# lujiarui/esmdiff

Hardware: AMD Instinct MI355X
Metric: conformation samples/sec (256-res, 25 steps) (higher is better)
Workload: dtype bf16

## Files before the change

esmdiff_amd/_native.py:

```python
from __future__ import annotations

import ctypes
from pathlib import Path

import os

_LIB_PATH = Path(os.environ.get("ESMDIFF_LIB") or Path(__file__).resolve().parent / "lib" / "libesmdiff_hip.so")
_lib = None

c_f32p = ctypes.POINTER(ctypes.c_float)
c_i64p = ctypes.POINTER(ctypes.c_int64)

EPI_BF16, EPI_RESID_F32, EPI_SWIGLU_BF16, EPI_BIAS_GELU_BF16, EPI_BIAS_F32 = range(5)
DT_F32, DT_BF16 = 0, 1
PRECISION = {"bf16": 0, "f32": 1, "f32_split": 2, "f16": 3}
F32EPI_STORE, F32EPI_BIAS_GELU, F32EPI_RESID_DIV = range(3)
SECTIONS = ["embed", "layernorm", "gemm_qkv", "qk_norm_rope", "attention", "gemm_out", "gemm_ffn_up",
            "gemm_ffn_down", "head", "sampler"]


class Config(ctypes.Structure):
    _fields_ = [("d_model", ctypes.c_int32), ("n_heads", ctypes.c_int32), ("n_layers", ctypes.c_int32),
                ("ffn_hidden", ctypes.c_int32), ("vocab_out", ctypes.c_int32), ("freq_dim", ctypes.c_int32),
                ("max_batch", ctypes.c_int32), ("max_len", ctypes.c_int32), ("residue_scale", ctypes.c_float),
# ... 29 lines not shown
    "esmdiff_attention_f16", "esmdiff_qk_norm_rope", "esmdiff_add_layernorm", "esmdiff_geom_attention",
    "esmdiff_set_lengths", "esmdiff_attention_ragged", "esmdiff_attention_16_parts",
    "esmdiff_q_xt", "esmdiff_nelbo_rows", "esmdiff_nelbo_eval",
    "esmdiff_superpose_pairs", "esmdiff_tm_pairs",
    "esmdiff_cluster_threshold", "esmdiff_cluster_gromos",
    "esmdiff_lddt_pairs",
    "esmdiff_flex_pair_msf", "esmdiff_flex_fit", "esmdiff_flex_moments",
    "esmdiff_dssp",
    "esmdiff_contact_map", "esmdiff_native_contacts",
    "esmdiff_backbone_torsions", "esmdiff_ramachandran",
    "esmdiff_shape_frames", "esmdiff_debye_frames",
    "esmdiff_describe_gemm_choice", "esmdiff_gemm_workspace_floats",
    "esmdiff_dim6_to_backbone", "esmdiff_plddt_mean", "esmdiff_pair_features", "esmdiff_pae_tm",
    "esmdiff_decoder_set_pair_chunk_bytes",
    "esmdiff_encoder_knn", "esmdiff_encoder_neighbourhood", "esmdiff_encoder_nearest_code",
    "esmdiff_forward_logits_needed", "esmdiff_get_tail_rows",
    "esmdiff_layernorm_f32rows", "esmdiff_swiglu_f32", "esmdiff_qk_norm_rope_f32", "esmdiff_v_split",
    "esmdiff_attention_f32_parts", "esmdiff_gemm_split_k", "esmdiff_get_attention_scales",
    "esmdiff_convert_weight", "esmdiff_interleave_swiglu", "esmdiff_split_weight_from", "esmdiff_weight_rownorm_max",
    "esmdiff_embed_rows", "esmdiff_gather_table_rows", "esmdiff_sigma_mlp", "esmdiff_layernorm_16in",
    "esmdiff_mask_row_list", "esmdiff_gather_rows16", "esmdiff_add_layernorm_rows", "esmdiff_copy_masked_logits",
    "esmdiff_ddpm_step_mapped", "esmdiff_move_token_rows", "esmdiff_samples_with_mask", "esmdiff_rows_identical",
]
LDDT_MAX_L, LDDT_MAX_THRESHOLDS = 4096, 8
DSSP_MAX_L = 4096
TM_MAX_L = 1280
CONTACT_MAX_L, CONTACT_TILE, CONTACT_MAX_CHUNKS = 4096, 64, 256
RAMA_MAX_BINS = 72
SHAPE_MAX_L, SHAPE_MAX_BINS = 4096, 4096
DEBYE_MAX_Q, DEBYE_Q_CHUNK = 1024, 8

CLUSTER_MAX_N = 16384
QXT_PHILOX_COLUMN = 4104
OPT_STREAMS, OPT_DUAL_MIN_TOKENS, OPT_NEEDED_ROWS = 1, 2, 3


def flex_pair_slots(n: int) -> int:
    rows = (n + 1) // 2
    return 4 * rows * min(16, max(1, 2048 // rows))


def contact_pair_tiles(L: int) -> int:
    tiles = (L + CONTACT_TILE - 1) // CONTACT_TILE
    return tiles * (tiles + 1) // 2


def contact_chunk_frames(n: int, L: int) -> int:
    cap = min(CONTACT_MAX_CHUNKS, max(1, 1024 // contact_pair_tiles(L)))
    return max(16, (n + cap - 1) // cap)
# ... 43 lines not shown
            "esmdiff_amd has no CPU fallback.")
    L = ctypes.CDLL(str(_LIB_PATH))
    vp, i32, f32 = ctypes.c_void_p, ctypes.c_int32, ctypes.c_float
    L.esmdiff_abi_version.restype = ctypes.c_int
    L.esmdiff_engine_create.argtypes = [ctypes.POINTER(Config), ctypes.POINTER(Weight), i32, i32,
                                        ctypes.POINTER(vp)]
    L.esmdiff_engine_destroy.argtypes = [vp]
    L.esmdiff_engine_destroy.restype = None
    L.esmdiff_last_error.argtypes = [vp]
    L.esmdiff_last_error.restype = ctypes.c_char_p
    L.esmdiff_forward_logits.argtypes = [vp, vp, vp, vp, vp, i32, i32, i32, vp]
    L.esmdiff_forward_logits_sigmas.argtypes = [vp, vp, vp, vp, vp, i32, i32, i32, vp]
    L.esmdiff_forward_logits_sigmas.restype = ctypes.c_int
    L.esmdiff_forward_logits_needed.argtypes = [vp, vp, vp, vp, vp, i32, i32, i32, vp]
    L.esmdiff_get_tail_rows.argtypes = [vp, c_i64p, i32]
    L.esmdiff_ddpm_step.argtypes = [vp, vp, vp, i32, f32, f32, i32, vp, ctypes.POINTER(Rng), i32, i32, i32, vp]
    L.esmdiff_ddpm_step_margin.argtypes = [vp, vp, vp, i32, f32, f32, i32, ctypes.POINTER(Rng), i32, i32, i32, f32, vp, vp]
    L.esmdiff_ddpm_step_margin.restype = ctypes.c_int
    L.esmdiff_ddpm_step_rows.argtypes = [vp, vp, vp, i32, vp, ctypes.c_uint64, i32, i32, f32, f32, vp, vp, vp]
    L.esmdiff_logit_error_stats.argtypes = [vp, i32, vp, i32, vp, i32, i32, i32, vp, vp]
    L.esmdiff_gibbs_step_rows.argtypes = [vp, vp, vp, vp, i32, f32, f32, vp, ctypes.c_uint64, i32, i32, f32, f32, vp, vp, vp]
    L.esmdiff_get_build_info.argtypes = [ctypes.c_char_p, i32]
    L.esmdiff_describe_plan.argtypes = [vp, i32, i32, ctypes.c_char_p, i32]
    L.esmdiff_set_option.argtypes = [vp, i32, ctypes.c_int64]
    L.esmdiff_ddpm_sample.argtypes = [vp, vp, vp, i32, i32, i32, c_f32p, c_f32p, c_f32p, ctypes.POINTER(Rng), vp]
    L.esmdiff_gibbs_step.argtypes = [vp, vp, vp, vp, i32, f32, f32, vp, vp, ctypes.POINTER(Rng), i32, i32, i32, vp]
    L.esmdiff_gibbs_sample.argtypes = [vp, vp, vp, i32, i32, i32, f32, f32, ctypes.POINTER(i32), ctypes.POINTER(Rng), vp]
    L.esmdiff_gemm_bf16.argtypes = [vp, vp, vp, vp, i32, i32, i32, i32, i32, f32, i32, vp]
    L.esmdiff_gemm_f16.argtypes = [vp, vp, vp, vp, i32, i32, i32, i32, i32, f32, i32, vp]
    if hasattr(L, "esmdiff_gemm_bf16_timed"):
# ... 120 lines not shown
```

esmdiff_amd/csrc/engine.h:

```cpp
#pragma once
#include <math.h>
#include <stdarg.h>
#include <stdio.h>
#include <stdlib.h>
#include <string.h>

#include <algorithm>
#include <map>
#include <string>
#include <vector>

#include "kernels.h"
#define ed ed16
#include "kernels_typed.inc"
#undef ed

#define ED_KN(f16, call) ((f16) ? ed16::call : ed::call)

namespace eng {

enum Section { S_EMBED = 0, S_LN, S_QKV, S_QKROPE, S_ATTN, S_OUT, S_FFN_UP, S_FFN_DOWN, S_HEAD, S_SAMPLER, S_COUNT };

constexpr int64_t kDefaultPairChunkBytes = 1536ll << 20;

// ... 89 lines not shown
        *fmid = nullptr, *fpair_qk = nullptr;
  int step0_share = 0;
  int32_t* flag_dev = nullptr;
  int final_skip = 0;
  int32_t *has_dev = nullptr, *idx_dev = nullptr;
  int64_t *cx = nullptr, *cseq = nullptr;
  float* n_rowloss = nullptr;
  int g_strategy = 0;
  uint32_t* g_inv_mask = nullptr;
  bool g_inv_on = false;
  int needed_rows = 1;
  int32_t *rows_list = nullptr, *rows_map = nullptr, *rows_count = nullptr;
  hipEvent_t ev_rows = nullptr;
  bool rows_mapped = false;
  int64_t stat_tail_rows = 0;
  int64_t stat_forwards = 0, stat_rows = 0;
  int last_B = 0, last_L = 0;
  bool last_pending_delta = false;
  int profiling = 0;
  std::vector<hipEvent_t> ev;
  std::vector<int> ev_section;
  size_t ev_used = 0;
  float prof_ms[16] = {0};
  int prof_launches[16] = {0};
};

namespace eng {

int fail(Owner* o, int code, const char* fmt, ...);
const char* last_error(const Owner* o);
int round_up(int v, int m);
void softplus_host(float* v, int n);
int check_bl(esmdiff_engine* e, int B, int L);
int check_lens(esmdiff_engine* e, int B, int L);
int check_not_decoder(esmdiff_engine* e);
int forward(esmdiff_engine* e, const int64_t* seq, const int64_t* xtok, const float* t_freq_dev, float* logits, int ld, int B, int L,
            hipStream_t st, bool needed_rows = false);
int shared_forward_batch(const esmdiff_engine* e, int B, int L);

#define HIP_TRY(e, call)                                                                              \
  do {                                                                                                \
    hipError_t _s = (call);                                                                           \
    if (_s != hipSuccess) return eng::fail(e, ESMDIFF_E_HIP, "%s: %s", #call, hipGetErrorString(_s)); \
  } while (0)

template <typename T>
int dalloc(Owner* o, T** p, size_t n_elems, bool zero = false) {
  void* v = nullptr;
  hipError_t s = hipMalloc(&v, n_elems * sizeof(T) + 256);
  if (s != hipSuccess) return fail(o, ESMDIFF_E_HIP, "hipMalloc(%zu): %s", n_elems * sizeof(T), hipGetErrorString(s));
  if (zero) hipMemset(v, 0, n_elems * sizeof(T) + 256);
  o->allocs.push_back(v);
// ... 49 lines not shown
```

esmdiff_amd/csrc/engine.hip:

```cpp
#include "engine.h"

using namespace ed;
using namespace eng;

namespace {

thread_local std::string g_error;

}

namespace eng {

int fail(Owner* o, int code, const char* fmt, ...) {
  char buf[512];
  va_list ap;
  va_start(ap, fmt);
  vsnprintf(buf, sizeof buf, fmt, ap);
  va_end(ap);
  if (o) o->err = buf; else g_error = buf;
  return code;
}

const char* last_error(const Owner* o) { return o ? o->err.c_str() : g_error.c_str(); }

// ... 121 lines not shown
    case ESMDIFF_OPT_STREAMS:
      if (value < 1 || value > 4) return fail(e, ESMDIFF_E_INVALID, "ESMDIFF_OPT_STREAMS: 1 .. 4, got %lld", (long long)value);
      HIP_TRY(e, hipSetDevice(e->device));
      while ((int64_t)e->side.size() + 1 < value)
        if (int r = add_side_stream(e)) return r;
      e->n_streams = (int)value;
      return 0;
    case ESMDIFF_OPT_DUAL_MIN_TOKENS:
      if (value < 1) return fail(e, ESMDIFF_E_INVALID, "ESMDIFF_OPT_DUAL_MIN_TOKENS must be positive");
      e->dual_min_tokens = value;
      return 0;
    case ESMDIFF_OPT_NEEDED_ROWS:
      if (value != 0 && value != 1) return fail(e, ESMDIFF_E_INVALID, "ESMDIFF_OPT_NEEDED_ROWS: 0 or 1, got %lld", (long long)value);
      e->needed_rows = (int)value;
      return 0;
    default:
      return fail(e, ESMDIFF_E_INVALID, "unknown option %d", option);
  }
}

int esmdiff_get_build_info(char* buf, int32_t cap) {
#ifdef ED_DEBUG
  const int dbg = 1;
#else
  const int dbg = 0;
#endif
  char tmp[512];
  const int n = snprintf(tmp, sizeof tmp,
                         "libesmdiff_hip abi=%d arch=gfx950 debug_env=%d (%s) operand_builds=bf16,f16 fp_contract_off=sampler,gibbs,metrics "
                         "compiler=%s",
// ... 23 lines not shown
  return 0;
}

int esmdiff_get_counters(esmdiff_engine* e, int64_t* forwards, int64_t* token_rows, int32_t reset) {
  if (!e) return ESMDIFF_E_INVALID;
  if (forwards) *forwards = e->stat_forwards;
  if (token_rows) *token_rows = e->stat_rows;
  if (reset) e->stat_forwards = e->stat_rows = 0;
  return 0;
}

int esmdiff_get_tail_rows(esmdiff_engine* e, int64_t* rows_out, int32_t reset) {
  if (!e) return ESMDIFF_E_INVALID;
  if (rows_out) *rows_out = e->stat_tail_rows;
  if (reset) e->stat_tail_rows = 0;
  return 0;
}

int esmdiff_abi_version(void) { return ESMDIFF_ABI_VERSION; }

const char* esmdiff_last_error(const esmdiff_engine* eng) { return last_error(eng); }

void esmdiff_engine_destroy(esmdiff_engine* e) {
  if (!e) return;
  hipSetDevice(e->device);
  hipDeviceSynchronize();
  for (void* p : e->allocs) hipFree(p);
  for (void* p : {(void*)e->pair_x, (void*)e->pair_h, (void*)e->pair_logits})
    if (p) hipFree(p);
  for (hipEvent_t ev : e->ev) hipEventDestroy(ev);
// ... 258 lines not shown
      TRY(dalloc(e, &e->f_trans, Mx * 3));
      TRY(dalloc(e, &e->f_mask, Mx));
    }
    if (!strict) TRY(dalloc(e, &e->mid, Mx * FH));
    TRY(dalloc(e, &e->logits, Mx * e->ld_logits));
    if (e->has_plddt) TRY(dalloc(e, &e->pl_logits, Mx * e->ld_plddt));
    if (e->has_pair) {
      if (!strict) TRY(dalloc(e, &e->pair_qk, Mx * 128));
      TRY(dalloc(e, &e->tm_rows, Mx));
      TRY(dalloc(e, &e->ptm_dev, (size_t)cfg->max_batch));
    }
    TRY(dalloc(e, &e->cond, (size_t)cfg->max_batch * D));
    TRY(dalloc(e, &e->sig_hidden, (size_t)cfg->max_batch * D));
    e->tfreq_rows = 1026;
    TRY(dalloc(e, &e->tfreq, (size_t)e->tfreq_rows * F));
    TRY(dalloc(e, &e->g_entropy, Mx));
    TRY(dalloc(e, &e->flag_dev, (size_t)4));
    TRY(dalloc(e, &e->has_dev, (size_t)cfg->max_batch));
    TRY(dalloc(e, &e->idx_dev, (size_t)cfg->max_batch));
    TRY(dalloc(e, &e->lens_dev, (size_t)cfg->max_batch));
    TRY(dalloc(e, &e->lens_sub_dev, (size_t)cfg->max_batch));
    TRY(dalloc(e, &e->cx, Mx));
    TRY(dalloc(e, &e->cseq, Mx));
    TRY(dalloc(e, &e->n_rowloss, Mx));
    TRY(dalloc(e, &e->g_inv_mask, (size_t)128, true));
    TRY(dalloc(e, &e->g_sampled, Mx));
    TRY(dalloc(e, &e->g_rowflag, Mx));
    TRY(dalloc(e, &e->g_rowgap, Mx));
    TRY(dalloc(e, &e->g_nunmask, (size_t)e->tfreq_rows * cfg->max_batch));
    {
// ... 116 lines not shown
```

esmdiff_amd/csrc/engine_forward.hip:

```cpp
#include "engine.h"

using namespace ed;
using namespace eng;

namespace {

struct Part {
  const int64_t *seq, *xtok;
  float *x, *logits, *pl_logits;
  bf16_t *h, *h2, *qkv, *q, *k, *ctx, *mid, *dlt, *dlt2, *gp, *gctx, *pair_qk;
  float *fh, *fh2, *fqkv, *fq, *fk, *fctx, *fgu, *fmid, *fgp, *fgctx, *fpair_qk;
  uint16_t* a2;
  float* rs;
  const float *f_rot, *f_trans;
  const uint8_t* f_mask;
  const int32_t* lens;
  int b0, B;
  hipStream_t st;
  const GemmWorkspace *gws, *gws2;
};

void cut_batch(esmdiff_engine* e, Part* parts, int np, const int64_t* seq, const int64_t* xtok, float* logits, int ld, int B, int L,
               hipStream_t st) {
  const int64_t D = e->cfg.d_model, FH = e->cfg.ffn_hidden, VH = e->v_heads;
// ... 295 lines not shown
const char kStaleRows[] =
    "the last forward ran inside esmdiff_ddpm_sample on the rows that hold MASK only (ESMDIFF_OPT_NEEDED_ROWS): the other rows' "
    "hidden state is stale; run a full forward (esmdiff_forward_logits) first, or set the option to 0";

}

int eng::shared_forward_batch(const esmdiff_engine* e, int B, int L) {
  if (e->strict) return 1;
  if (plan_small(e, B, L)) return B;
  for (int b = 1; b < B; ++b)
    if (!plan_small(e, b, L) && (int64_t)b * L >= ed::small_max_rows()) return b;
  return B;
}

int eng::forward(esmdiff_engine* e, const int64_t* seq, const int64_t* xtok, const float* t_freq_dev, float* logits,
                 int ld, int B, int L, hipStream_t st, bool needed_rows) {
  e->last_B = B;
  e->last_L = L;
  e->last_pending_delta = false;
  e->rows_mapped = false;
  e->stat_forwards += 1;
  e->stat_rows += (int64_t)B * L;
  if (e->has_geom && e->frames_B > 0 && (e->frames_B != B || e->frames_L != L))
    return fail(e, ESMDIFF_E_INVALID, "frames were set for B=%d L=%d, forward called with B=%d L=%d", e->frames_B, e->frames_L, B, L);
  const int D = e->cfg.d_model;
  Prof p{e, st};
  const float* cond = nullptr;
  if (t_freq_dev && e->sig_w1) {
    RUN(S_EMBED, launch_sigma_mlp(t_freq_dev, e->sig_w1, e->sig_b1, e->sig_w2, e->sig_b2, e->sig_hidden, e->cond, e->cfg.freq_dim, D, st,
                                  e->sigma_rows));
    cond = e->cond;
  }
  const BatchPlan plan = plan_batch(e, B, L);
  Part parts[4];
  cut_batch(e, parts, plan.np, seq, xtok, logits, ld, B, L, st);
  bool needed = needed_rows && e->needed_rows && e->rows_count && !e->head_split && !plan.small && !e->has_plddt && !e->has_pair &&
                e->cfg.n_layers >= 2;
  if (needed) {
    hipStreamCaptureStatus cs = hipStreamCaptureStatusNone;
    HIP_TRY(e, hipStreamIsCapturing(st, &cs));
    needed = cs == hipStreamCaptureStatusNone;
  }
  if (needed) {
    HIP_TRY(e, launch_mask_row_list(xtok, B, L, plan.np, e->rows_list, e->rows_map, e->rows_count, st));
    HIP_TRY(e, hipEventRecord(e->ev_rows, st));
  }
  if (int r = fork_streams(e, st, plan.np)) return r;
  if (e->strict) {
    for (int pi = 0; pi < plan.np; ++pi)
      if (int r = strict_part(e, parts[pi], cond && e->sigma_rows > 1 ? cond + (int64_t)parts[pi].b0 * D : cond, ld, L)) return r;
  } else if (int r = forward_16bit(e, parts, plan, cond, ld, L, needed)) {
    return r;
  }
  if (!needed) e->stat_tail_rows += (int64_t)B * L;
  return join_streams(e, st, plan.np);
}

extern "C" {

int esmdiff_describe_plan(const esmdiff_engine* e, int32_t B, int32_t L, char* buf, int32_t cap) {
  if (!e || B <= 0 || L <= 0) return ESMDIFF_E_INVALID;
  const esmdiff_config& c = e->cfg;
  const int D = c.d_model, FH = c.ffn_hidden;
  char tmp[1536];
  int n = 0;
  auto room = [&]() { return n < (int)sizeof tmp ? sizeof tmp - (size_t)n : (size_t)0; };
  auto at = [&]() { return tmp + (n < (int)sizeof tmp ? n : (int)sizeof tmp - 1); };
  const char* prec = e->strict ? (e->split ? "f32_split" : "f32") : (e->f16 ? "f16" : "bf16");
  n += snprintf(at(), room(), "precision=%s head=%s B=%d L=%d", prec, (e->strict || e->head_split) ? "f32-grade" : prec, B, L);
  const int np = plan_parts(e, B, L);
// ... 7 lines not shown
    char g1[32], g2[32], g3[32], g4[32];
    const size_t wsf = e->gemm_ws[0].partial ? e->gemm_ws[0].partial_floats : 0;
    ed::describe_gemm(m0, 3 * D, D, wsf, g1, sizeof g1);
    ed::describe_gemm(m0, D, D, wsf, g2, sizeof g2);
    ed::describe_gemm(m0, 2 * FH, D, wsf, g3, sizeof g3);
    ed::describe_gemm(m0, D, FH, 0, g4, sizeof g4);
    n += snprintf(at(), room(), " streams=%d rows_per_stream=%d path=%s", np, m0, small ? "small-batch(K-slice planes summed by the LayerNorm)" : "regular");
    if (small)
      n += snprintf(at(), room(), " gemm[qkv]=%s gemm[out]=128x*/S%d gemm[ffn_up]=%s gemm[ffn_down]=128x*/S%d", g1, ed::gemm_partial_splits(D, D), g3,
                    ed::gemm_partial_splits(D, FH));
    else
      n += snprintf(at(), room(), " gemm[qkv]=%s gemm[out]=%s gemm[ffn_up]=%s gemm[ffn_down]=%s", g1, g2, g3, g4);
  }
  n += snprintf(at(), room(), " step0_sharing=%d final_skip=%d small_max_rows=%d needed_rows=%d", e->step0_share, e->final_skip,
                ed::small_max_rows(), e->needed_rows);
  if (e->lens_B == B) {
    int64_t valid = 0;
    for (int b = 0; b < B; ++b) valid += std::min<int64_t>(e->lens_host[b], L);
    n += snprintf(at(), room(), " ragged=1 valid_tokens=%lld padded_tokens=%lld", (long long)valid, (long long)B * L);
  }
  if (buf && cap > 0) snprintf(buf, (size_t)cap, "%s", tmp);
  return n;
}

int esmdiff_shared_forward_batch(const esmdiff_engine* e, int32_t B, int32_t L) {
  if (!e || B <= 0 || L <= 0 || B > e->cfg.max_batch || L > e->cfg.max_len) return ESMDIFF_E_INVALID;
  return shared_forward_batch(e, B, L);
}

int esmdiff_forward_logits(esmdiff_engine* e, const int64_t* seq, const int64_t* x, const float* t_freq,
// ... 71 lines not shown
```

esmdiff_amd/csrc/engine_sample.hip:

```cpp
#include "engine.h"

using namespace ed;
using namespace eng;

namespace {

int step0_shared_batch(esmdiff_engine* e, const int64_t* seq, const int64_t* x, int B, int L, hipStream_t st, int* shared) {
  *shared = 0;
  if (!e->step0_share || B < 2) return 0;
  if (e->frames_B != 0) return 0;
  if (e->lens_B != 0) return 0;
  const int bs = shared_forward_batch(e, B, L);
  if (bs >= B) return 0;
  HIP_TRY(e, launch_rows_identical(seq, x, B, L, e->flag_dev, st));
  int32_t h = 0;
  HIP_TRY(e, hipMemcpyAsync(&h, e->flag_dev, sizeof h, hipMemcpyDeviceToHost, st));
  HIP_TRY(e, hipStreamSynchronize(st));
  if (h != 0) *shared = bs;
  return 0;
}

int check_mask_head(esmdiff_engine* e, const char* who) {
  return e->cfg.vocab_out <= ESMDIFF_MASK_ID ? fail(e, ESMDIFF_E_INVALID, "%s needs the 4101-way head (mask column)", who) : 0;
}
// ... 123 lines not shown
                        void* stream) {
  if (!e) return ESMDIFF_E_INVALID;
  if (int r = check_not_decoder(e)) return r;
  if (!seq || !x_inout || !mc_t || !mc_s || !rng) return fail(e, ESMDIFF_E_INVALID, "null pointer");
  if (T <= 0 || T + 1 > e->tfreq_rows) return fail(e, ESMDIFF_E_INVALID, "num_steps %d out of range (1..%d)", T, e->tfreq_rows - 1);
  if (e->cfg.time_conditioning && !t_freq) return fail(e, ESMDIFF_E_INVALID, "t_freq required with time conditioning");
  if (int r = check_bl(e, B, L)) return r;
  if (int r = check_lens(e, B, L)) return r;
  hipStream_t st = (hipStream_t)stream;
  const int F = e->cfg.freq_dim;
  if (t_freq) {
    e->tfreq_host.assign(t_freq, t_freq + (size_t)(T + 1) * F);
    HIP_TRY(e, hipMemcpyAsync(e->tfreq, e->tfreq_host.data(), e->tfreq_host.size() * sizeof(float), hipMemcpyHostToDevice, st));
  }
  Prof p{e, st};
  int shared = 0;
  if (int r = step0_shared_batch(e, seq, x_inout, B, L, st, &shared)) return r;
  for (int i = 0; i <= T; ++i) {
    const int Bf = (i == 0 && shared) ? shared : B;
    if (i == T && e->final_skip && T > 0) {
      HIP_TRY(e, launch_samples_with_mask(x_inout, B, L, e->has_dev, st));
      std::vector<int32_t> has(B);
      HIP_TRY(e, hipMemcpyAsync(has.data(), e->has_dev, (size_t)B * 4, hipMemcpyDeviceToHost, st));
      HIP_TRY(e, hipStreamSynchronize(st));
      std::vector<int32_t> idx;
      for (int b = 0; b < B; ++b)
        if (has[b]) idx.push_back(b);
      const int n_live = (int)idx.size();
      if (n_live == 0) break;
      const int n_min = shared_forward_batch(e, B, L);
      if (n_min < B && n_live < B) {
        for (int b = 0; (int)idx.size() < n_min && b < B; ++b)
          if (!has[b]) idx.push_back(b);
        const int n_run = (int)idx.size();
        HIP_TRY(e, hipMemcpyAsync(e->idx_dev, idx.data(), (size_t)n_run * 4, hipMemcpyHostToDevice, st));
        HIP_TRY(e, launch_move_token_rows(x_inout, e->cx, e->idx_dev, n_run, L, 1, st));
        HIP_TRY(e, launch_move_token_rows(seq, e->cseq, e->idx_dev, n_run, L, 1, st));
        std::vector<int32_t> sub_lens;
        if (e->lens_B) {
          for (int j = 0; j < n_run; ++j) sub_lens.push_back(e->lens_host[idx[j]]);
          HIP_TRY(e, hipMemcpyAsync(e->lens_sub_dev, sub_lens.data(), (size_t)n_run * 4, hipMemcpyHostToDevice, st));
          e->cur_lens = e->lens_sub_dev;
        }
        const int rf = forward(e, e->cseq, e->cx, t_freq ? e->tfreq + (size_t)i * F : nullptr, e->logits, e->ld_logits, n_run, L, st, true);
        e->cur_lens = e->lens_B ? e->lens_dev : nullptr;
        if (rf) return rf;
        RUN(S_SAMPLER, launch_ddpm_step(e->cx, e->logits, e->ld_logits, e->cfg.vocab_out, 0.f, 0.f, 1, nullptr, 1, rng->seed, rng->sample_offset, i, n_run, L, st, 0,
                                        0.f, nullptr, e->rows_mapped ? e->rows_map : nullptr));
        HIP_TRY(e, launch_move_token_rows(e->cx, x_inout, e->idx_dev, n_live, L, 0, st));
        HIP_TRY(e, hipStreamSynchronize(st));
        break;
      }
    }
    if (int r = forward(e, seq, x_inout, t_freq ? e->tfreq + (size_t)i * F : nullptr, e->logits, e->ld_logits, Bf, L, st, true)) return r;
    const int fin = i == T;
    RUN(S_SAMPLER, launch_ddpm_step(x_inout, e->logits, e->ld_logits, e->cfg.vocab_out, fin ? 0.f : mc_t[i], fin ? 0.f : mc_s[i],
                                    fin, nullptr, 1, rng->seed, rng->sample_offset, i, B, L, st, Bf < B ? Bf : 0, 0.f, nullptr,
                                    e->rows_mapped ? e->rows_map : nullptr));
  }
  return 0;
}

int esmdiff_gibbs_step(esmdiff_engine* e, int64_t* x_inout, const int64_t* seq, const float* logits, int32_t ld_logits,
                       float temperature, float top_p, const int32_t* n_unmask, const float* u, const esmdiff_rng* rng,
                       int32_t step, int32_t B, int32_t L, void* stream) {
  if (!e) return ESMDIFF_E_INVALID;
  if (!x_inout || !seq || !logits || !n_unmask) return fail(e, ESMDIFF_E_INVALID, "null pointer");
  if (!u && !rng) return fail(e, ESMDIFF_E_INVALID, "need explicit uniforms or an rng");
  if (int r = check_gibbs_filter(e, temperature, top_p, &ld_logits)) return r;
  if (int r = check_bl(e, B, L)) return r;
  if (e->g_strategy == 1 && u) return fail(e, ESMDIFF_E_INVALID, "strategy \"random\" draws its positions from the Philox source: pass rng, not explicit uniforms");
  Prof p{e, (hipStream_t)stream};
  RUN(S_SAMPLER, launch_gibbs_step(x_inout, seq, logits, ld_logits, e->cfg.vocab_out, temperature, top_p, n_unmask, u, u ? 0 : 1, rng ? rng->seed : 0,
// ... 52 lines not shown
```

esmdiff_amd/csrc/kernels.h:

```cpp
#pragma once
#include <stdlib.h>
#include <hip/hip_runtime.h>
#include <stdint.h>

#include "../../include/esmdiff_hip.h"
#include "../../include/esmdiff_hip_test.h"

#include <map>
#include <mutex>
#include <utility>

typedef uint16_t bf16_t;

struct EdGemmWorkspace {
  float* partial;
  size_t partial_floats;
};
struct EdGemmPartials {
  const float* p;
  int S;
  int64_t stride;
};

inline int finish_entry(hipStream_t st) {
// ... 19 lines not shown

hipError_t launch_ddpm_step(int64_t* x, const float* logits, int ld, int V, float mc_t, float mc_s, int final_,
                            const float* u, int use_philox, uint64_t seed, uint64_t sample_offset, int step,
                            int B, int L, hipStream_t stream, int logits_period = 0, float margin = 0.f,
                            int32_t* sample_flags = nullptr, const int32_t* row_map = nullptr);
hipError_t launch_ddpm_step_rows(int64_t* x, const float* logits, int ld, int V, const esmdiff_sample_step* sp, uint64_t seed,
                                 int B, int L, float margin_ratio, float margin_diff, int32_t* sample_flags, float* sample_gap,
                                 hipStream_t stream);
hipError_t launch_logit_error_stats(const float* a, int lda, const float* b, int ldb, const int64_t* x, int rows, int V, int all_columns,
                                    float* out, hipStream_t stream);
hipError_t launch_samples_with_mask(const int64_t* x, int B, int L, int32_t* has, hipStream_t stream);
hipError_t launch_move_token_rows(const int64_t* src, int64_t* dst, const int32_t* idx, int n, int L, int gather, hipStream_t stream);
hipError_t launch_rows_identical(const int64_t* seq, const int64_t* x, int B, int L, int32_t* flag, hipStream_t stream);
__host__ __device__ inline bool needed_rows_compact(int count, int rows) { return (int64_t)count * 8 <= (int64_t)rows * 7; }
hipError_t launch_mask_row_list(const int64_t* x, int B, int L, int np, int32_t* list, int32_t* map, int32_t* count_host,
                                hipStream_t stream);
hipError_t launch_gather_rows16(const uint16_t* src, const int32_t* list, uint16_t* dst, int n, int D, hipStream_t stream);
hipError_t launch_copy_masked_logits(const int64_t* x, const float* logits, int ld, const int32_t* map, float* out, int ld_out,
                                     int V, int rows, hipStream_t stream);

hipError_t launch_q_xt(const int64_t* x0, const int64_t* seq, const float* move_chance, const uint8_t* non_moving, const float* u,
                       uint64_t seed, const uint64_t* sample_index, const int32_t* draw, const int32_t* lens, int64_t* xt,
                       int64_t* seq_out, int B, int L, hipStream_t stream);
hipError_t launch_nelbo_rows(const float* logits, int ld, int V, const int64_t* xt, const int64_t* x0, const float* weight,
                             const uint8_t* loss_mask, const int32_t* lens, float* log_p, float* row_loss, float* sample_sum,
                             int32_t* sample_count, int B, int L, hipStream_t stream);

hipError_t launch_gibbs_step(int64_t* x, const int64_t* seq, const float* logits, int ld, int vocab, float temperature,
                             float top_p, const int32_t* n_unmask, const float* u, int use_philox, uint64_t seed,
                             uint64_t sample_offset, int step, int32_t* sampled, float* entropy, int B, int L,
                             hipStream_t stream, int logits_period = 0, int strategy = 0, const uint32_t* inv_mask = nullptr);
// ... 57 lines not shown
```

esmdiff_amd/csrc/sampler.hip:

```cpp
#include "ed_math.h"
#include "ed_wave.h"
#include "kernels.h"

namespace ed {

constexpr int NT = 256;
constexpr int MASK_ID = ESMDIFF_MASK_ID;
constexpr int MAX_PER_THREAD = 20;

template <int PER, bool MARGIN = false, bool ROWS = false, bool MAPPED = false>
__global__ __launch_bounds__(NT) void ddpm_step_kernel(int64_t* __restrict__ x, const float* __restrict__ logits,
                                                       int ld, int V, float mc_t, float mc_s, int final_,
                                                       const float* __restrict__ u, int use_philox,
                                                       uint64_t seed, uint64_t sample_offset, int step, int L,
                                                       int logits_period, float margin = 0.f,
                                                       int32_t* __restrict__ sample_flags = nullptr,
                                                       const esmdiff_sample_step* __restrict__ sp = nullptr,
                                                       float margin_fin = 0.f, float* __restrict__ sample_gap = nullptr,
                                                       const int32_t* __restrict__ row_map = nullptr) {
  const int row = blockIdx.x;
  if (x[row] != MASK_ID) return;
  uint64_t sample_index = 0;
  if constexpr (ROWS) {
    const esmdiff_sample_step q = sp[row / L];
// ... 335 lines not shown
    __syncthreads();
    int before = 0, tile = 0;
    for (int w = 0; w < RL_NT / 64; ++w) {
      before += w < wave ? s_wave[w] : 0;
      tile += s_wave[w];
    }
    if (on) {
      const int i = base + before + __popcll(bal & ((1ull << lane) - 1ull));
      list[t0 + i] = r;
      map[t0 + r] = t0 + (compact ? i : r);
    }
    base += tile;
  }
}

hipError_t launch_mask_row_list(const int64_t* x, int B, int L, int np, int32_t* list, int32_t* map, int32_t* count_host,
                                hipStream_t stream) {
  if (B <= 0 || L <= 0 || np <= 0 || np > B) return hipErrorInvalidValue;
  hipLaunchKernelGGL(mask_row_list_kernel, dim3(np), dim3(RL_NT), 0, stream, x, B, L, np, list, map, count_host);
  return hipGetLastError();
}

__global__ __launch_bounds__(256) void gather_rows16_kernel(const uint16_t* __restrict__ src, const int32_t* __restrict__ list,
                                                            uint16_t* __restrict__ dst, int n, int D) {
  const int i = blockIdx.x * 4 + (threadIdx.x >> 6), lane = threadIdx.x & 63;
  if (i >= n) return;
  const uint4* s = reinterpret_cast<const uint4*>(src + (int64_t)list[i] * D);
  uint4* d = reinterpret_cast<uint4*>(dst + (int64_t)i * D);
  for (int c = lane; c < D / 8; c += 64) d[c] = s[c];
}

hipError_t launch_gather_rows16(const uint16_t* src, const int32_t* list, uint16_t* dst, int n, int D, hipStream_t stream) {
  if (n <= 0) return hipSuccess;
  if (D <= 0 || D % 8 != 0) return hipErrorInvalidValue;
// ... 31 lines not shown
```

esmdiff_amd/engine.py:

```python
from __future__ import annotations

import ctypes
import contextlib
from typing import Dict, Optional, Sequence

import torch

from . import _native as N
from .config import ModelConfig
from .constants import SEQUENCE_PAD_TOKEN, STRUCTURE_MASK_TOKEN, STRUCTURE_PAD_TOKEN, STRUCTURE_VOCAB
from .schedule import DDPMSchedule


def _ptr(t: Optional[torch.Tensor]):
    return ctypes.c_void_p(0 if t is None else t.data_ptr())


def _stream() -> ctypes.c_void_p:
    return ctypes.c_void_p(torch.cuda.current_stream().cuda_stream)


def _require_gpu():
    if not torch.cuda.is_available():
        raise RuntimeError("esmdiff_amd needs an MI355X (gfx950) GPU: torch.cuda.is_available() is False and "
# ... 531 lines not shown
    def shared_forward_batch(self, B: int, L: int) -> int:
        n = self._lib.esmdiff_shared_forward_batch(self._h, int(B), int(L))
        if n < 0:
            self._chk(n)
        return int(n)

    def set_small_batch_splitk(self, on: bool) -> None:
        self._chk(self._lib.esmdiff_set_small_batch_splitk(self._h, int(bool(on))))

    def set_final_skip(self, on: bool) -> None:
        self._chk(self._lib.esmdiff_set_final_skip(self._h, int(bool(on))))

    def set_needed_rows(self, on: bool) -> None:
        self._chk(self._lib.esmdiff_set_option(self._h, N.OPT_NEEDED_ROWS, int(bool(on))))

    def forward_logits_needed(self, x: torch.Tensor, sequence_tokens: torch.Tensor, t_freq: Optional[torch.Tensor],
                              out: torch.Tensor) -> torch.Tensor:
        B, L = x.shape
        x, seq = self._tok(x, B, L), self._tok(sequence_tokens, B, L)
        tf = None if t_freq is None else t_freq.to(device=self.device, dtype=torch.float32).contiguous()
        self._chk(self._lib.esmdiff_forward_logits_needed(self._h, _ptr(seq), _ptr(x), _ptr(tf), _ptr(out), out.shape[-1], B, L, _stream()))
        return out

    def tail_rows(self, reset: bool = False) -> int:
        r = ctypes.c_int64(0)
        self._chk(self._lib.esmdiff_get_tail_rows(self._h, ctypes.byref(r), int(reset)))
        return int(r.value)

    def counters(self, reset: bool = False) -> Dict[str, int]:
        f, r = ctypes.c_int64(0), ctypes.c_int64(0)
# ... 643 lines not shown
```

include/esmdiff_hip.h:

```cpp
#ifndef ESMDIFF_HIP_H
#define ESMDIFF_HIP_H

#include <stdint.h>

#ifdef __cplusplus
extern "C" {
#endif

#define ESMDIFF_ABI_VERSION 8

#define ESMDIFF_VOCAB 4101
#define ESMDIFF_MASK_ID 4096
#define ESMDIFF_STRUCT_EOS 4097
#define ESMDIFF_STRUCT_BOS 4098
#define ESMDIFF_STRUCT_PAD 4099
#define ESMDIFF_STRUCT_CHAINBREAK 4100

typedef enum {
  ESMDIFF_OK = 0,
  ESMDIFF_E_INVALID = -1,
  ESMDIFF_E_MISSING = -2,
  ESMDIFF_E_SHAPE = -3,
  ESMDIFF_E_HIP = -4,
  ESMDIFF_E_CAPACITY = -5,
// ... 29 lines not shown

typedef struct {
  uint64_t seed;
  uint64_t sample_offset;
} esmdiff_rng;

#define ESMDIFF_QXT_PHILOX_COLUMN 4104

typedef struct esmdiff_engine esmdiff_engine;

int esmdiff_abi_version(void);

int esmdiff_get_build_info(char* buf, int32_t cap);
int esmdiff_describe_plan(const esmdiff_engine* eng, int32_t B, int32_t L, char* buf, int32_t cap);

typedef enum { ESMDIFF_OPT_STREAMS = 1, ESMDIFF_OPT_DUAL_MIN_TOKENS = 2, ESMDIFF_OPT_NEEDED_ROWS = 3 } esmdiff_option;
int esmdiff_set_option(esmdiff_engine* eng, int32_t option, int64_t value);

int esmdiff_engine_create(const esmdiff_config* cfg, const esmdiff_weight* table, int32_t n,
                          int32_t device, esmdiff_engine** out);
void esmdiff_engine_destroy(esmdiff_engine* eng);

const char* esmdiff_last_error(const esmdiff_engine* eng);

int esmdiff_forward_logits(esmdiff_engine* eng, const int64_t* seq, const int64_t* x,
                           const float* t_freq, float* logits_out, int32_t ld_logits,
                           int32_t B, int32_t L, void* stream);

int esmdiff_forward_logits_sigmas(esmdiff_engine* eng, const int64_t* seq, const int64_t* x, const float* t_freq,
                                  float* logits_out, int32_t ld_logits, int32_t B, int32_t L, void* stream);

// ... 187 lines not shown
```

Before: 59.68.

## Precompute sigma conditioning table and optionally run DDPM update per sub-batch stream

Computes the sigma-MLP conditioning for all timesteps once before the sampling loop and passes a per-step slice into forward, removing one small MLP launch per step. Adds an opt-in mode that runs the DDPM sampling update and the next step's mask-row listing on each sub-batch stream before the streams join. This lets sampling of one part overlap with the remaining forward work of other parts, at the cost of more launches and extra per-part bookkeeping. Launch counters are added for diagnosis.

```diff
diff --git a/esmdiff_amd/_native.py b/esmdiff_amd/_native.py
--- a/esmdiff_amd/_native.py
+++ b/esmdiff_amd/_native.py
@@ -67,7 +67,7 @@
     "esmdiff_dim6_to_backbone", "esmdiff_plddt_mean", "esmdiff_pair_features", "esmdiff_pae_tm",
     "esmdiff_decoder_set_pair_chunk_bytes",
     "esmdiff_encoder_knn", "esmdiff_encoder_neighbourhood", "esmdiff_encoder_nearest_code",
-    "esmdiff_forward_logits_needed", "esmdiff_get_tail_rows",
+    "esmdiff_forward_logits_needed", "esmdiff_get_tail_rows", "esmdiff_get_sampler_launches",
     "esmdiff_layernorm_f32rows", "esmdiff_swiglu_f32", "esmdiff_qk_norm_rope_f32", "esmdiff_v_split",
     "esmdiff_attention_f32_parts", "esmdiff_gemm_split_k", "esmdiff_get_attention_scales",
     "esmdiff_convert_weight", "esmdiff_interleave_swiglu", "esmdiff_split_weight_from", "esmdiff_weight_rownorm_max",
@@ -85,7 +85,7 @@
 
 CLUSTER_MAX_N = 16384
 QXT_PHILOX_COLUMN = 4104
-OPT_STREAMS, OPT_DUAL_MIN_TOKENS, OPT_NEEDED_ROWS = 1, 2, 3
+OPT_STREAMS, OPT_DUAL_MIN_TOKENS, OPT_NEEDED_ROWS, OPT_SAMPLER_PER_PART = 1, 2, 3, 4
 
 
 def flex_pair_slots(n: int) -> int:
@@ -159,6 +159,7 @@
     L.esmdiff_forward_logits_sigmas.restype = ctypes.c_int
     L.esmdiff_forward_logits_needed.argtypes = [vp, vp, vp, vp, vp, i32, i32, i32, vp]
     L.esmdiff_get_tail_rows.argtypes = [vp, c_i64p, i32]
+    L.esmdiff_get_sampler_launches.argtypes = [vp, c_i64p, i32]
     L.esmdiff_ddpm_step.argtypes = [vp, vp, vp, i32, f32, f32, i32, vp, ctypes.POINTER(Rng), i32, i32, i32, vp]
     L.esmdiff_ddpm_step_margin.argtypes = [vp, vp, vp, i32, f32, f32, i32, ctypes.POINTER(Rng), i32, i32, i32, f32, vp, vp]
     L.esmdiff_ddpm_step_margin.restype = ctypes.c_int
diff --git a/esmdiff_amd/csrc/engine.h b/esmdiff_amd/csrc/engine.h
--- a/esmdiff_amd/csrc/engine.h
+++ b/esmdiff_amd/csrc/engine.h
@@ -127,6 +127,9 @@
   hipEvent_t ev_rows = nullptr;
   bool rows_mapped = false;
   int64_t stat_tail_rows = 0;
+  float *cond_table = nullptr, *sig_hidden_table = nullptr;
+  int sampler_per_part = 0;
+  int64_t stat_sampler[4] = {0, 0, 0, 0};
   int64_t stat_forwards = 0, stat_rows = 0;
   int last_B = 0, last_L = 0;
   bool last_pending_delta = false;
@@ -147,8 +150,19 @@
 int check_bl(esmdiff_engine* e, int B, int L);
 int check_lens(esmdiff_engine* e, int B, int L);
 int check_not_decoder(esmdiff_engine* e);
+struct DdpmForward {
+  const float* cond = nullptr;
+  bool update = false;
+  int64_t* x = nullptr;
+  float mc_t = 0.f, mc_s = 0.f;
+  int fin = 0, step = 0;
+  uint64_t seed = 0, sample_offset = 0;
+  bool list_next = false;
+  bool rows_ready = false;
+  bool sampled = false, listed = false;
+};
 int forward(esmdiff_engine* e, const int64_t* seq, const int64_t* xtok, const float* t_freq_dev, float* logits, int ld, int B, int L,
-            hipStream_t st, bool needed_rows = false);
+            hipStream_t st, bool needed_rows = false, DdpmForward* ddpm = nullptr);
 int shared_forward_batch(const esmdiff_engine* e, int B, int L);
 
 #define HIP_TRY(e, call)                                                                              \
diff --git a/esmdiff_amd/csrc/engine.hip b/esmdiff_amd/csrc/engine.hip
--- a/esmdiff_amd/csrc/engine.hip
+++ b/esmdiff_amd/csrc/engine.hip
@@ -159,6 +159,10 @@
       if (value != 0 && value != 1) return fail(e, ESMDIFF_E_INVALID, "ESMDIFF_OPT_NEEDED_ROWS: 0 or 1, got %lld", (long long)value);
       e->needed_rows = (int)value;
       return 0;
+    case ESMDIFF_OPT_SAMPLER_PER_PART:
+      if (value != 0 && value != 1) return fail(e, ESMDIFF_E_INVALID, "ESMDIFF_OPT_SAMPLER_PER_PART: 0 or 1, got %lld", (long long)value);
+      e->sampler_per_part = (int)value;
+      return 0;
     default:
       return fail(e, ESMDIFF_E_INVALID, "unknown option %d", option);
   }
@@ -212,6 +216,15 @@
   if (!e) return ESMDIFF_E_INVALID;
   if (rows_out) *rows_out = e->stat_tail_rows;
   if (reset) e->stat_tail_rows = 0;
+  return 0;
+}
+
+int esmdiff_get_sampler_launches(esmdiff_engine* e, int64_t* out4, int32_t reset) {
+  if (!e) return ESMDIFF_E_INVALID;
+  for (int i = 0; i < 4; ++i) {
+    if (out4) out4[i] = e->stat_sampler[i];
+    if (reset) e->stat_sampler[i] = 0;
+  }
   return 0;
 }
 
@@ -500,6 +513,8 @@
     TRY(dalloc(e, &e->sig_hidden, (size_t)cfg->max_batch * D));
     e->tfreq_rows = 1026;
     TRY(dalloc(e, &e->tfreq, (size_t)e->tfreq_rows * F));
+    TRY(dalloc(e, &e->cond_table, (size_t)e->tfreq_rows * D));
+    TRY(dalloc(e, &e->sig_hidden_table, (size_t)e->tfreq_rows * D));
     TRY(dalloc(e, &e->g_entropy, Mx));
     TRY(dalloc(e, &e->flag_dev, (size_t)4));
     TRY(dalloc(e, &e->has_dev, (size_t)cfg->max_batch));
diff --git a/esmdiff_amd/csrc/engine_forward.hip b/esmdiff_amd/csrc/engine_forward.hip
--- a/esmdiff_amd/csrc/engine_forward.hip
+++ b/esmdiff_amd/csrc/engine_forward.hip
@@ -333,7 +333,7 @@
 }
 
 int eng::forward(esmdiff_engine* e, const int64_t* seq, const int64_t* xtok, const float* t_freq_dev, float* logits,
-                 int ld, int B, int L, hipStream_t st, bool needed_rows) {
+                 int ld, int B, int L, hipStream_t st, bool needed_rows, DdpmForward* ddpm) {
   e->last_B = B;
   e->last_L = L;
   e->last_pending_delta = false;
@@ -345,7 +345,9 @@
   const int D = e->cfg.d_model;
   Prof p{e, st};
   const float* cond = nullptr;
-  if (t_freq_dev && e->sig_w1) {
+  if (ddpm && ddpm->cond) {
+    cond = ddpm->cond;
+  } else if (t_freq_dev && e->sig_w1) {
     RUN(S_EMBED, launch_sigma_mlp(t_freq_dev, e->sig_w1, e->sig_b1, e->sig_w2, e->sig_b2, e->sig_hidden, e->cond, e->cfg.freq_dim, D, st,
                                   e->sigma_rows));
     cond = e->cond;
@@ -355,14 +357,17 @@
   cut_batch(e, parts, plan.np, seq, xtok, logits, ld, B, L, st);
   bool needed = needed_rows && e->needed_rows && e->rows_count && !e->head_split && !plan.small && !e->has_plddt && !e->has_pair &&
                 e->cfg.n_layers >= 2;
-  if (needed) {
+  bool per_part = ddpm && ddpm->update && e->sampler_per_part && plan.np > 1 && !e->strict;
+  if (needed || per_part) {
     hipStreamCaptureStatus cs = hipStreamCaptureStatusNone;
     HIP_TRY(e, hipStreamIsCapturing(st, &cs));
-    needed = cs == hipStreamCaptureStatusNone;
-  }
-  if (needed) {
+    needed = needed && cs == hipStreamCaptureStatusNone;
+    per_part = per_part && cs == hipStreamCaptureStatusNone;
+  }
+  if (needed && !(ddpm && ddpm->rows_ready)) {
     HIP_TRY(e, launch_mask_row_list(xtok, B, L, plan.np, e->rows_list, e->rows_map, e->rows_count, st));
     HIP_TRY(e, hipEventRecord(e->ev_rows, st));
+    e->stat_sampler[2] += 1;
   }
   if (int r = fork_streams(e, st, plan.np)) return r;
   if (e->strict) {
@@ -372,7 +377,28 @@
     return r;
   }
   if (!needed) e->stat_tail_rows += (int64_t)B * L;
-  return join_streams(e, st, plan.np);
+  if (per_part) {
+    for (int pi = 0; pi < plan.np; ++pi) {
+      const Part& w = parts[pi];
+      const int64_t t0 = (int64_t)w.b0 * L;
+      p.s = w.st;
+      RUN(S_SAMPLER, launch_ddpm_step(ddpm->x + t0, e->rows_mapped ? logits : w.logits, ld, e->cfg.vocab_out, ddpm->mc_t, ddpm->mc_s,
+                                      ddpm->fin, nullptr, 1, ddpm->seed, ddpm->sample_offset + (uint64_t)w.b0, ddpm->step, w.B, L, w.st,
+                                      0, 0.f, nullptr, e->rows_mapped ? e->rows_map + t0 : nullptr));
+    }
+    ddpm->sampled = true;
+    e->stat_sampler[1] += 1;
+    if (needed && ddpm->list_next) {
+      for (int pi = 0; pi < plan.np; ++pi)
+        HIP_TRY(e, launch_mask_row_list(ddpm->x, B, L, plan.np, e->rows_list, e->rows_map, e->rows_count, parts[pi].st, pi));
+      ddpm->listed = true;
+      e->stat_sampler[3] += 1;
+    }
+    p.s = st;
+  }
+  if (int r = join_streams(e, st, plan.np)) return r;
+  if (ddpm && ddpm->listed) HIP_TRY(e, hipEventRecord(e->ev_rows, st));
+  return 0;
 }
 
 extern "C" {
@@ -410,6 +436,7 @@
   }
   n += snprintf(at(), room(), " step0_sharing=%d final_skip=%d small_max_rows=%d needed_rows=%d", e->step0_share, e->final_skip,
                 ed::small_max_rows(), e->needed_rows);
+  n += snprintf(at(), room(), " ddpm_update=%s", (e->sampler_per_part && np > 1 && !e->strict) ? "per-sub-batch" : "whole-batch");
   if (e->lens_B == B) {
     int64_t valid = 0;
     for (int b = 0; b < B; ++b) valid += std::min<int64_t>(e->lens_host[b], L);
diff --git a/esmdiff_amd/csrc/engine_sample.hip b/esmdiff_amd/csrc/engine_sample.hip
--- a/esmdiff_amd/csrc/engine_sample.hip
+++ b/esmdiff_amd/csrc/engine_sample.hip
@@ -161,8 +161,13 @@
     HIP_TRY(e, hipMemcpyAsync(e->tfreq, e->tfreq_host.data(), e->tfreq_host.size() * sizeof(float), hipMemcpyHostToDevice, st));
   }
   Prof p{e, st};
+  const bool table = t_freq && e->sig_w1;
+  const int D = e->cfg.d_model;
+  if (table)
+    RUN(S_EMBED, launch_sigma_mlp(e->tfreq, e->sig_w1, e->sig_b1, e->sig_w2, e->sig_b2, e->sig_hidden_table, e->cond_table, F, D, st, T + 1));
   int shared = 0;
   if (int r = step0_shared_batch(e, seq, x_inout, B, L, st, &shared)) return r;
+  bool rows_ready = false;
   for (int i = 0; i <= T; ++i) {
     const int Bf = (i == 0 && shared) ? shared : B;
     if (i == T && e->final_skip && T > 0) {
@@ -189,21 +194,39 @@
           HIP_TRY(e, hipMemcpyAsync(e->lens_sub_dev, sub_lens.data(), (size_t)n_run * 4, hipMemcpyHostToDevice, st));
           e->cur_lens = e->lens_sub_dev;
         }
-        const int rf = forward(e, e->cseq, e->cx, t_freq ? e->tfreq + (size_t)i * F : nullptr, e->logits, e->ld_logits, n_run, L, st, true);
+        DdpmForward df;
+        df.cond = table ? e->cond_table + (size_t)i * D : nullptr;
+        const int rf = forward(e, e->cseq, e->cx, t_freq ? e->tfreq + (size_t)i * F : nullptr, e->logits, e->ld_logits, n_run, L, st, true, &df);
         e->cur_lens = e->lens_B ? e->lens_dev : nullptr;
         if (rf) return rf;
         RUN(S_SAMPLER, launch_ddpm_step(e->cx, e->logits, e->ld_logits, e->cfg.vocab_out, 0.f, 0.f, 1, nullptr, 1, rng->seed, rng->sample_offset, i, n_run, L, st, 0,
                                         0.f, nullptr, e->rows_mapped ? e->rows_map : nullptr));
+        e->stat_sampler[0] += 1;
         HIP_TRY(e, launch_move_token_rows(e->cx, x_inout, e->idx_dev, n_live, L, 0, st));
         HIP_TRY(e, hipStreamSynchronize(st));
         break;
       }
     }
-    if (int r = forward(e, seq, x_inout, t_freq ? e->tfreq + (size_t)i * F : nullptr, e->logits, e->ld_logits, Bf, L, st, true)) return r;
     const int fin = i == T;
-    RUN(S_SAMPLER, launch_ddpm_step(x_inout, e->logits, e->ld_logits, e->cfg.vocab_out, fin ? 0.f : mc_t[i], fin ? 0.f : mc_s[i],
+    DdpmForward df;
+    df.cond = table ? e->cond_table + (size_t)i * D : nullptr;
+    df.update = Bf == B;
+    df.x = x_inout;
+    df.mc_t = fin ? 0.f : mc_t[i];
+    df.mc_s = fin ? 0.f : mc_s[i];
+    df.fin = fin;
+    df.step = i;
+    df.seed = rng->seed;
+    df.sample_offset = rng->sample_offset;
+    df.list_next = i < T && !(i + 1 == T && e->final_skip);
+    df.rows_ready = rows_ready;
+    if (int r = forward(e, seq, x_inout, t_freq ? e->tfreq + (size_t)i * F : nullptr, e->logits, e->ld_logits, Bf, L, st, true, &df)) return r;
+    rows_ready = df.listed;
+    if (df.sampled) continue;
+    RUN(S_SAMPLER, launch_ddpm_step(x_inout, e->logits, e->ld_logits, e->cfg.vocab_out, df.mc_t, df.mc_s,
                                     fin, nullptr, 1, rng->seed, rng->sample_offset, i, B, L, st, Bf < B ? Bf : 0, 0.f, nullptr,
                                     e->rows_mapped ? e->rows_map : nullptr));
+    e->stat_sampler[0] += 1;
   }
   return 0;
 }
diff --git a/esmdiff_amd/csrc/kernels.h b/esmdiff_amd/csrc/kernels.h
--- a/esmdiff_amd/csrc/kernels.h
+++ b/esmdiff_amd/csrc/kernels.h
@@ -57,7 +57,7 @@
 hipError_t launch_rows_identical(const int64_t* seq, const int64_t* x, int B, int L, int32_t* flag, hipStream_t stream);
 __host__ __device__ inline bool needed_rows_compact(int count, int rows) { return (int64_t)count * 8 <= (int64_t)rows * 7; }
 hipError_t launch_mask_row_list(const int64_t* x, int B, int L, int np, int32_t* list, int32_t* map, int32_t* count_host,
-                                hipStream_t stream);
+                                hipStream_t stream, int part = -1);
 hipError_t launch_gather_rows16(const uint16_t* src, const int32_t* list, uint16_t* dst, int n, int D, hipStream_t stream);
 hipError_t launch_copy_masked_logits(const int64_t* x, const float* logits, int ld, const int32_t* map, float* out, int ld_out,
                                      int V, int rows, hipStream_t stream);
diff --git a/esmdiff_amd/csrc/sampler.hip b/esmdiff_amd/csrc/sampler.hip
--- a/esmdiff_amd/csrc/sampler.hip
+++ b/esmdiff_amd/csrc/sampler.hip
@@ -373,10 +373,56 @@
   }
 }
 
+__global__ __launch_bounds__(RL_NT) void mask_row_list_part_kernel(const int64_t* __restrict__ x, int B, int L, int np, int pi,
+                                                                   int32_t* __restrict__ list, int32_t* __restrict__ map,
+                                                                   int32_t* __restrict__ count_host) {
+  __shared__ int s_wave[RL_NT / 64];
+  __shared__ int s_total;
+  const int t = threadIdx.x, lane = t & 63, wave = t >> 6;
+  const int t0 = (int)((int64_t)B * pi / np) * L, rows = (int)((int64_t)B * (pi + 1) / np) * L - t0;
+  const int64_t* xp = x + t0;
+  int n = 0;
+  for (int r = t; r < rows; r += RL_NT) n += xp[r] == MASK_ID;
+  n = wave_sum(n);
+  if (lane == 0) s_wave[wave] = n;
+  __syncthreads();
+  if (t == 0) {
+    int tot = 0;
+    for (int w = 0; w < RL_NT / 64; ++w) tot += s_wave[w];
+    s_total = tot;
+    count_host[pi] = tot;
+  }
+  __syncthreads();
+  const bool compact = needed_rows_compact(s_total, rows);
+  int base = 0;
+  for (int r0 = 0; r0 < rows; r0 += RL_NT) {
+    const int r = r0 + t;
+    const bool on = r < rows && xp[r] == MASK_ID;
+    const unsigned long long bal = __ballot(on);
+    __syncthreads();
+    if (lane == 0) s_wave[wave] = __popcll(bal);
+    __syncthreads();
+    int before = 0, tile = 0;
+    for (int w = 0; w < RL_NT / 64; ++w) {
+      before += w < wave ? s_wave[w] : 0;
+      tile += s_wave[w];
+    }
+    if (on) {
+      const int i = base + before + __popcll(bal & ((1ull << lane) - 1ull));
+      list[t0 + i] = r;
+      map[t0 + r] = t0 + (compact ? i : r);
+    }
+    base += tile;
+  }
+}
+
 hipError_t launch_mask_row_list(const int64_t* x, int B, int L, int np, int32_t* list, int32_t* map, int32_t* count_host,
-                                hipStream_t stream) {
-  if (B <= 0 || L <= 0 || np <= 0 || np > B) return hipErrorInvalidValue;
-  hipLaunchKernelGGL(mask_row_list_kernel, dim3(np), dim3(RL_NT), 0, stream, x, B, L, np, list, map, count_host);
+                                hipStream_t stream, int part) {
+  if (B <= 0 || L <= 0 || np <= 0 || np > B || part >= np) return hipErrorInvalidValue;
+  if (part >= 0)
+    hipLaunchKernelGGL(mask_row_list_part_kernel, dim3(1), dim3(RL_NT), 0, stream, x, B, L, np, part, list, map, count_host);
+  else
+    hipLaunchKernelGGL(mask_row_list_kernel, dim3(np), dim3(RL_NT), 0, stream, x, B, L, np, list, map, count_host);
   return hipGetLastError();
 }
 
diff --git a/esmdiff_amd/engine.py b/esmdiff_amd/engine.py
--- a/esmdiff_amd/engine.py
+++ b/esmdiff_amd/engine.py
@@ -569,6 +569,14 @@
     def set_needed_rows(self, on: bool) -> None:
         self._chk(self._lib.esmdiff_set_option(self._h, N.OPT_NEEDED_ROWS, int(bool(on))))
 
+    def set_sampler_per_part(self, on: bool) -> None:
+        self._chk(self._lib.esmdiff_set_option(self._h, N.OPT_SAMPLER_PER_PART, int(bool(on))))
+
+    def sampler_launches(self, reset: bool = False) -> Dict[str, int]:
+        v = (ctypes.c_int64 * 4)()
+        self._chk(self._lib.esmdiff_get_sampler_launches(self._h, v, int(reset)))
+        return {"update_whole": int(v[0]), "update_parts": int(v[1]), "list_whole": int(v[2]), "list_parts": int(v[3])}
+
     def forward_logits_needed(self, x: torch.Tensor, sequence_tokens: torch.Tensor, t_freq: Optional[torch.Tensor],
                               out: torch.Tensor) -> torch.Tensor:
         B, L = x.shape
diff --git a/include/esmdiff_hip.h b/include/esmdiff_hip.h
--- a/include/esmdiff_hip.h
+++ b/include/esmdiff_hip.h
@@ -67,7 +67,12 @@
 int esmdiff_get_build_info(char* buf, int32_t cap);
 int esmdiff_describe_plan(const esmdiff_engine* eng, int32_t B, int32_t L, char* buf, int32_t cap);
 
-typedef enum { ESMDIFF_OPT_STREAMS = 1, ESMDIFF_OPT_DUAL_MIN_TOKENS = 2, ESMDIFF_OPT_NEEDED_ROWS = 3 } esmdiff_option;
+typedef enum {
+  ESMDIFF_OPT_STREAMS = 1,
+  ESMDIFF_OPT_DUAL_MIN_TOKENS = 2,
+  ESMDIFF_OPT_NEEDED_ROWS = 3,
+  ESMDIFF_OPT_SAMPLER_PER_PART = 4
+} esmdiff_option;
 int esmdiff_set_option(esmdiff_engine* eng, int32_t option, int64_t value);
 
 int esmdiff_engine_create(const esmdiff_config* cfg, const esmdiff_weight* table, int32_t n,
```

After: 59.75 (median of 4 runs). About the same (+0.1%).
